# intel/QAT-ZSTD-Plugin

Measured on AMD Instinct MI355X. Metric: input MB/s via ZSTD_compress2 L1 128KiB blocks @1/2/4/8 GPU; ratio vs sw zstd, higher is better.
Workload: dtype u8

## Files before the change

include/qzstd_hip.h:

```cpp
#ifndef QZSTD_HIP_H
#define QZSTD_HIP_H

#include <stddef.h>
#include <stdint.h>

#if defined(__cplusplus)
extern "C" {
#endif

#define QZSTD_HIP_BLOCK_MAX (1u << 17)
#define QZSTD_HIP_NSEQ_ERROR 0xFFFFFFFFu
#define QZSTD_HIP_SRC_ALIGN 16u

typedef struct {
    uint32_t tableSize;
    uint32_t tileLog;
    uint32_t capLen;
    uint32_t minMatch;
    uint32_t farLog1;
    uint32_t farLog2;
    uint32_t lazy;
    uint32_t backExt;
    uint32_t nearTab;
    uint32_t window;
// ... 54 lines not shown
int qzstd_hip_stream_sync(int device, void *stream);
int qzstd_hip_stream_query(int device, void *stream);
int qzstd_hip_stream_wait(int device, void *stream, unsigned timeoutMs);
int qzstd_hip_memcpy_h2d(int device, void *stream, void *dst, const void *src, size_t bytes);
int qzstd_hip_copy_in(int device, void *stream, void *dst, const void *src_dev, size_t bytes);
int qzstd_hip_memcpy_d2h(int device, void *stream, void *dst, const void *src, size_t bytes);
int qzstd_hip_memset(int device, void *stream, void *dst, int value, size_t bytes);
int qzstd_hip_memcpy2d_d2h(int device, void *stream, void *dst, size_t dpitch, const void *src, size_t spitch,
                           size_t width, size_t height);

size_t qzstd_hip_workspace_bytes(int level, uint32_t nBlocks, uint32_t maxBlockLen);
int qzstd_hip_find_sequences(int device, void *stream, int level, const void *d_src,
                             const qzstd_hip_block_t *d_blocks, uint32_t nBlocks,
                             uint32_t maxBlockLen, void *d_seqs, uint32_t *d_nseq,
                             void *d_work, size_t workBytes);

int qzstd_hip_occupancy(int device, int level);

#define QZSTD_HIP_NSEQ_REJECTED 0xFFFFFFFEu
#define QZSTD_HIP_NSEQ_STAGING 0xFFFFFFFCu
int qzstd_hip_service_progressive(int device);
#define QZSTD_HIP_SVC_MAX_ITEMS 32u
#define QZSTD_HIP_SVC_MAX_SLOTS 1024u
typedef struct {
    const void *hSrc;
    void *dSrc;
    void *hSeqs;
    uint32_t *hCount;
    uint32_t srcLen, itemBytes, nItems, seqCapPerItem;
    uint32_t slot;
// ... 25 lines not shown
```

qat-zstd-plugin_amd/csrc/qzstd_kernels.hip:

```cpp
#include <hip/hip_runtime.h>

#include <stdint.h>
#include <stdio.h>
#include <stdlib.h>
#include <string.h>

#include <atomic>
#include <mutex>
#include <sched.h>
#include <time.h>

#include "qzstd_hip.h"
#include "qzstd_hip_internal.h"

#define QZ_PRIO(n) do { if (!CHAIN) __builtin_amdgcn_s_setprio(n); } while (0)

#ifndef QZ_PARSE_SPLIT
#define QZ_PARSE_SPLIT 3
#endif
#ifndef QZ_LINKS_PER_STEP
#define QZ_LINKS_PER_STEP 4
#endif
#ifndef QZ_WAVES_PER_EU
#define QZ_WAVES_PER_EU 5
#endif
#define QZ_OCCUPANCY __attribute__((amdgpu_waves_per_eu(QZ_WAVES_PER_EU)))

#ifdef QZ_DEBUG_DUMP
#define QZ_PLAP(acc) { const u64 tN = __builtin_amdgcn_s_memtime(); acc += tN - tQ; tQ = tN; }
#define QZ_LAP(acc) { const u64 tN = __builtin_amdgcn_s_memtime(); acc += tN - tP; tP = tN; }
#define QZ_CLAP(k) { const u64 tN = __builtin_amdgcn_s_memtime(); dC[k] += tN - tC; tC = tN; }
#else
#define QZ_PLAP(acc)
#define QZ_LAP(acc)
#define QZ_CLAP(k)
#endif

namespace {

constexpr int kMatchWaves = 8;
constexpr int kMatchThreads = kMatchWaves * 64;
// ... 689 lines not shown
}

struct HistShare {
    uint32_t *flags;
    uint32_t item;
    uint32_t epoch;
    uint32_t spinLimit;
    uint32_t nItems;
    uint32_t *tabFlags;
    uint32_t *linkFlags;
    uint32_t *tabs;
};
constexpr uint32_t kSvcTabStride = QZ_CHAIN_TABLE;
static_assert((uint32_t)kMatchWaves * kPvStride <= QZ_CHAIN_TABLE, "the deferred parse's eight windows of parse words must fit in the head table (QZ_CHAIN_TABLE)");

template <bool HAS_LONG, bool REP, bool CHAIN, bool TURNS, bool NEAR, bool DEFER = false>
__device__ __forceinline__ uint32_t qz_item(const LaunchArgs &args, const qzstd_hip_block_t &blk, const uint8_t *gsrc, uint4 *out,
                                            uint4 *chainB, uint32_t *p1B, const HistShare hsh)
{
    extern __shared__ __attribute__((aligned(16))) uint8_t smem[];
    const uint32_t tid = threadIdx.x;
    const uint32_t lane = tid & 63u;
    const uint32_t wave = rdfirst(tid >> 6);
    const bool matcher = wave < (uint32_t)kMatchWaves;
    const uint32_t n = blk.srcLen;
    const qzstd_hip_profile_t pf = args.prof;
    const uint32_t nh = n >= pf.hashBytes ? n - pf.hashBytes + 1u : 0u;
    const uint32_t nTiles = (nh + kTile - 1u) >> kTileLog;
    const uint32_t itEnd = (DEFER && !CHAIN) ? nTiles : nTiles + kLagT;
    static_assert(kNear + kLagT * kTile + 4u <= kRing - kLook, "the ring no longer holds a near source when its tile is parsed / emitted");
    const uint32_t tabShift = (uint32_t)__builtin_clz(pf.tableSize) + 1u, longShift = pf.longSize ? (uint32_t)__builtin_clz(pf.longSize) + 1u : 31u;
    const uint32_t firstTile = blk.parseFrom >> kTileLog;
    if (blk.parseFrom != 0u && (pf.segLog == 0u || (blk.parseFrom & ((1u << pf.segLog) - 1u)) != 0u || blk.parseFrom >= n)) {
        return QZSTD_HIP_NSEQ_ERROR;
    }
    if (NEAR && n > kRing) return QZSTD_HIP_NSEQ_ERROR;
    if (DEFER && args.pwWords != 0u && ((n + kTile - 1u) & ~(kTile - 1u)) > args.pwWords) return QZSTD_HIP_NSEQ_ERROR;
    if (DEFER && CHAIN && args.chainEntries != 0u && ((n + kTile - 1u) & ~(kTile - 1u)) * kEQ > args.chainEntries) return QZSTD_HIP_NSEQ_ERROR;

    uint8_t *smemI = (uint8_t *)(__attribute__((address_space(3))) uint8_t *)kLdsBase;
    if ((uint32_t)(uintptr_t)(__attribute__((address_space(3))) uint8_t *)smem != 0u) {
        return QZSTD_HIP_NSEQ_ERROR;
    }
    uint32_t *ring32 = reinterpret_cast<uint32_t *>(smemI);
    uint4 *ring128 = reinterpret_cast<uint4 *>(smemI);
    uint32_t *tbl = reinterpret_cast<uint32_t *>(smemI + kRing + kMirror);
    uint32_t *tblL = tbl + pf.tableSize;
    uint32_t *nearTab = tblL + pf.longSize;
    uint32_t *srec = nearTab + kTile;
    uint32_t *pv = srec + kLagT * kWin * kSrecWords;
    uint32_t *turnCtr = pv + kLagT * kPvStride;
    uint32_t *P1odd = turnCtr + QZSTD_HIP_LDS_CTRL / 4u;
    const uint4 *g128 = reinterpret_cast<const uint4 *>(gsrc);
    Src src;
    src.ring = (LdsWords)ring32;
    src.g = (HbmWords)reinterpret_cast<const uint32_t *>(gsrc);
    src.nearLimit = NEAR ? 0xFFFFFFFFu : kNear;
    const uint32_t nPad = (n + 15u) & ~15u;

    const uint32_t itBegin = firstTile;
    const uint32_t histEnd = itBegin << kTileLog;
    const uint32_t hi = umin(nPad, histEnd + kLook + (itBegin ? 0u : kTile));
    const uint32_t lo = hi > kRing ? (hi - kRing + 15u) & ~15u : 0u;
    constexpr uint32_t kStep = (uint32_t)kThreads * 16u;
    const uint32_t hashEnd = CHAIN ? 0u : histEnd;
    uint32_t fo = (hashEnd ? 0u : lo) + tid * 16u;
    uint4 fa0 = make_uint4(0u, 0u, 0u, 0u), fb0 = fa0, fa1 = fa0, fb1 = fa0;
    if (fo < hi) { fa0 = g128[fo >> 4]; if (fo < hashEnd) fb0 = g128[(fo >> 4) + 1u]; }
    if (fo + kStep < hi) { fa1 = g128[(fo + kStep) >> 4]; if (fo + kStep < hashEnd) fb1 = g128[((fo + kStep) >> 4) + 1u]; }
    for (uint32_t i = tid; i < pf.tableSize + pf.longSize; i += kThreads) tbl[i] = 0u;
    if (!(CHAIN && itBegin != 0u)) {
        for (uint32_t i = tid; i < kTile; i += kThreads) nearTab[i] = 0xFFFFFFFFu;
        for (uint32_t i = tid; i < kLagT * kWin * kSrecWords + kLagT * kPvStride + QZSTD_HIP_LDS_CTRL / 4u; i += kThreads) srec[i] = 0u;
    }
    const bool sharedHist = CHAIN && hsh.flags != nullptr && hsh.nItems > 1u && pf.tableSize <= kSvcTabStride;
    if (itBegin != 0u || sharedHist) __syncthreads();
    if (sharedHist) {
        constexpr uint32_t kGroup = 4096u;
        uint32_t *hist = ring32;
        uint32_t *link = ring32 + kGroup;
        const uint32_t a0 = blk.parseFrom, b0 = n, k = hsh.item;
        auto wait_for = [&](uint32_t *fl) -> bool {
            if (wave == 0u) {
                uint32_t spins = 0u, ok = 1u;
// ... 229 lines not shown
                __builtin_amdgcn_fence(__ATOMIC_ACQUIRE, "agent");
                if (lane == 0u) turnCtr[2] = ok;
            }
            __syncthreads();
            if (rdfirst(turnCtr[2]) == 0u) return QZSTD_HIP_NSEQ_ERROR;
        }
        __syncthreads();
        for (uint32_t i = tid; i < kTile; i += kThreads) nearTab[i] = 0xFFFFFFFFu;
        for (uint32_t i = tid; i < kLagT * kWin * kSrecWords + kLagT * kPvStride + QZSTD_HIP_LDS_CTRL / 4u; i += kThreads) srec[i] = 0u;
    }
    {
        const uint32_t hiMaskH = pf.hashBytes >= 8 ? 0xFFFFFFFFu : ((1u << (8u * (pf.hashBytes - 4u))) - 1u);
        for (; fo < hi; fo += kStep) {
            uint4 fa2 = make_uint4(0u, 0u, 0u, 0u), fb2 = fa2;
            const uint32_t o2 = fo + 2u * kStep;
            if (o2 < hi) { fa2 = g128[o2 >> 4]; if (o2 < hashEnd) fb2 = g128[(o2 >> 4) + 1u]; }
            if (fo >= lo) {
                const uint32_t r = ring_dw(fo) << 2;
                ring128[r >> 4] = fa0;
                if (r < kMirror) ring128[(kRing + r) >> 4] = fa0;
            }
            if (fo < hashEnd) {
                const uint32_t W[6] = { fa0.x, fa0.y, fa0.z, fa0.w, fb0.x, fb0.y };
                const uint32_t segEc = seg_end(pf, fo, n);
#pragma unroll
                for (uint32_t k = 0; k < 16u; k++) {
                    const uint32_t p = fo + k;
                    if (p + pf.hashBytes <= segEc) {
                        const uint32_t v = __builtin_amdgcn_alignbyte(W[(k >> 2) + 1u], W[k >> 2], k & 3u);
                        const uint32_t w = __builtin_amdgcn_alignbyte(W[(k >> 2) + 2u], W[(k >> 2) + 1u], k & 3u);
                        const uint32_t mixH = (v * kPrime1) ^ __umul24(pf.hashBytes > 4 ? w & hiMaskH : 0u, kPrime2 & 0xFFFFFFu);
                        atomicMax(&tbl[mixH >> tabShift], ((p + 1u) << kTagBits) | ((mixH >> 3) & kTagMask));
                        if (HAS_LONG && p + 8u <= segEc) {
                            const uint32_t m8 = (v * kPrime1) ^ (w * kPrime2);
                            atomicMax(&tblL[m8 >> longShift], ((p + 1u) << kTagBits) | ((m8 >> 3) & kTagMask));
                        }
                    }
                }
            }
            fa0 = fa1; fb0 = fb1; fa1 = fa2; fb1 = fb2;
        }
        if (itBegin != 0u && TURNS && !CHAIN && tid == 0u) *turnCtr = itBegin * (uint32_t)kMatchWaves;
        if (itBegin == 0u)
            for (uint32_t o = hi + tid * 16u; o < kTile + kLook; o += kThreads * 16u) {
                ring128[o >> 4] = make_uint4(0u, 0u, 0u, 0u);
                if (o < kMirror) ring128[(kRing + o) >> 4] = make_uint4(0u, 0u, 0u, 0u);
            }
    }
    __syncthreads();

    if (DEFER && !matcher) __builtin_amdgcn_endpgm();
    if (!matcher) {
        if (!QZ_ABLATED(32u)) __builtin_amdgcn_s_setprio(3);
        constexpr uint32_t kSplit = QZ_PARSE_SPLIT;
#ifdef QZ_DEBUG_DUMP
        u64 pI1 = 0, pW1 = 0, pI2 = 0, pW2 = 0, tQ = __builtin_amdgcn_s_memtime();
#endif
        uint32_t nseqEnd, anchorEnd;
        if (REP) {
            RepState st = { blk.parseFrom, blk.parseFrom, 0u, 0u, 0u, 0u, pf.segLog ? blk.parseFrom >> pf.segLog : 0u };
            for (uint32_t it = itBegin; it < itEnd; it++) {
                const bool work = it >= 1u && it - 1u < nTiles && it - 1u >= firstTile && !QZ_ABLATED(1u);
                const uint32_t k = it - 1u, base = k << kTileLog;
// ... 99 lines not shown
            }
            const u64 startMask = __ballot(start);
            const uint32_t smLo = (uint32_t)startMask, smHi = (uint32_t)(startMask >> 32);
            const uint32_t keepLo = lane < 32u ? smLo & (0xFFFFFFFFu << (lane & 31u)) : 0u;
            const uint32_t keepHi = lane < 32u ? smHi : smHi & (0xFFFFFFFFu << (lane & 31u));
            const uint32_t ns = umin(umin(first_diff_bit(keepLo), first_diff_bit(keepHi) | 32u), 64u);
            const bool capped = cl == pf.capLen;
            const uint32_t endj = lane + cl;
            const uint32_t nsEnd = (uint32_t)__shfl((int)ns, (int)(endj & 63u));
            uint32_t nx = endj >= 64u ? endj : nsEnd;
            nx = capped ? kNxCapped : nx;
            const uint32_t gRep = take ? 4u * cl + 32u - (31u - (uint32_t)__builtin_clz(off + 1u)) : 0u;
            if (DEFER) p1B[(tileIdx << kTileLog) + tid] = gRep | (off << 10);
            else pv[(tileIdx % kLagT) * kPvStride + tid] = REP ? (gRep | (off << 10)) : pack_pos(nx, ns, capped ? off : cl);
    };
    for (uint32_t it = itBegin; it < itEnd; it++) {
        const uint32_t t0 = it << kTileLog;
        const uint32_t p = t0 + tid;
        const uint32_t stamp = (nTilesMax - 1u - (it & (nTilesMax - 1u))) << stampShift;
        uint32_t mix = 0, old = 0;
        const uint32_t segE = rdfirst(seg_end(pf, t0, n));
        const bool valid = it < nTiles && p < nh && p + pf.hashBytes <= segE;
        const bool history = it < firstTile;

        QZ_PRIO(2);
        if (CHAIN && DEFER && wave == 0u && it == itBegin && it < nTiles)
            chain_insert_tile(pf, src, tbl, (it & 1u) ? P1odd : nearTab, it << kTileLog, n, nh, lane, args.orderedLds != 0u);
        uint32_t own[5];
        load_dw_r<5>(src, p, rp, false, own);
        uint4 fresh;
        asm volatile("" : "=v"(fresh.x), "=v"(fresh.y), "=v"(fresh.z), "=v"(fresh.w));
        const uint32_t fpos = t0 + kLook + (tid - 64u) * 16u;
        const bool refill = wave == 1u && it >= 1u && lane < kTile / 16u && fpos < nPad;
        if (refill) fresh = g128[fpos >> 4];
        if (!DEFER && it >= kLagT + firstTile && !QZ_ABLATED(8u))
            emit_window<REP>(pf, src, srec + ((it % kLagT) * kWin + wave) * kSrecWords, pv + (it % kLagT) * kPvStride + 64u * wave,
                             offH[kLagT - 1u], lenH[kLagT - 1u], t0 - kLagT * kTile + 64u * wave, ring_back(rp, kLagT * kTile), lane, out, blk.seqCap,
                             REP ? srec[(it % kLagT) * kWin * kSrecWords] : 0u, blk.mark);
        QZ_PRIO(1);
        uint32_t slot = 0, nslot = 0, slotL = 0, oldL = 0, tagL = 0;
        const bool validL = HAS_LONG && valid && p + 8u <= segE;
        uint32_t oa[4];
#pragma unroll
        for (int i = 0; i < 4; i++) oa[i] = __builtin_amdgcn_alignbyte(own[i + 1], own[i], p & 3u);
        if (valid) {
            const uint32_t v = oa[0];
            uint32_t hi = 0;
            if (pf.hashBytes > 4) hi = oa[1] & hiMask;
// ... 6 lines not shown
                const uint32_t m8 = (v * kPrime1) ^ (oa[1] * kPrime2);
                slotL = m8 >> longShift;
                tagL = (m8 >> 3) & kTagMask;
                if (!TURNS) oldL = tblL[slotL];
            }
        }
        uint32_t pre[kEL];
#pragma unroll
        for (uint32_t j = 0; j < kEL; j++) pre[j] = 0u;
        if (CHAIN && it != itBegin) {
            old = valid ? ((it & 1u) ? P1odd : nearTab)[tid] : 0u;
            if (old != 0u && (old >> kTagBits) - 1u < t0) entryOf((old >> kTagBits) - 1u, pre);
        }
        if (CHAIN && it > itBegin && it - 1u < nTiles && it - 1u >= firstTile && !QZ_ABLATED(4u)) write_flags(it - 1u, lenH[0], offH[0]);
        QZ_LAP(dI1)
        __syncthreads();
        QZ_LAP(dW1)

        QZ_PRIO(2);
        if (CHAIN && DEFER && wave == 0u && it + 1u < nTiles)
            chain_insert_tile(pf, src, tbl, ((it + 1u) & 1u) ? P1odd : nearTab, (it + 1u) << kTileLog, n, nh, lane, args.orderedLds != 0u);
        if (refill) {
            const uint32_t o = ring_dw(fpos) << 2;
            ring128[o >> 4] = fresh;
            if (o < kMirror) ring128[(kRing + o) >> 4] = fresh;
        }
        uint32_t cl = 0, off = 0;
        if (CHAIN) {
            const uint32_t *P1T = (it & 1u) ? P1odd : nearTab;
            const uint32_t tag = (mix >> 3) & kTagMask;
#ifdef QZ_DEBUG_DUMP
            tC = __builtin_amdgcn_s_memtime();
#endif
            uint32_t E[kEL];
#pragma unroll
            for (uint32_t j = 0; j < kEL; j++) E[j] = 0u;
// ... 169 lines not shown
            }
            QZ_PRIO(0);
            l1 = umin(l1, cap); l2 = umin(l2, cap); l3 = umin(l3, cap);
            if (l1 >= 4u) { cl = l1; off = p - q1; }
            if (l3 >= 4u && l3 > cl) { cl = l3; off = p - q3; }
            if (l2 >= 4u && l2 >= cl) { cl = l2; off = p - q2; }
            }
        }
        }
        if (!CHAIN && it < nTiles && !history && !QZ_ABLATED(4u)) write_flags(it, cl, off);
#pragma unroll
        for (uint32_t i = kLagT - 1u; i > 0u; i--) { offH[i] = offH[i - 1u]; lenH[i] = lenH[i - 1u]; }
        offH[0] = off;
        lenH[0] = cl;
        rp = ring_fwd(rp, kTile);
        QZ_LAP(dI2)
        if (DEFER && !CHAIN) QZ_BARRIER_LDS(); else __syncthreads();
        QZ_LAP(dW2)
    }
#ifdef QZ_DEBUG_DUMP
    if (!(blk.mark & QZSTD_HIP_MARK_COMPACT)) {
    if (lane == 0) out[blk.seqCap - 3u - wave] = make_uint4((uint32_t)dI1, (uint32_t)dW1, (uint32_t)dI2, (uint32_t)dW2);
    if (lane == 0) out[blk.seqCap - 24u - 2u * wave] = make_uint4((uint32_t)(dC[0] >> 4), (uint32_t)(dC[1] >> 4), (uint32_t)(dC[2] >> 4), (uint32_t)(dC[3] >> 4));
    if (lane == 0) out[blk.seqCap - 25u - 2u * wave] = make_uint4((uint32_t)(dC[4] >> 4), (uint32_t)dC[5], 0u, 0u);
    if (lane == 0) out[blk.seqCap - 12u - wave] = make_uint4(__builtin_amdgcn_s_getreg((4 << 0) | (0 << 6) | (31 << 11)), 0u, 0u, 0u);
    }
#endif
    if constexpr (!DEFER) return 0u;
    }

    if constexpr (DEFER && !REP) {
        constexpr uint32_t kSegLog = 12u, kSeg = 1u << kSegLog, kMaxSegs = QZSTD_HIP_BLOCK_MAX >> kSegLog;
        static_assert(kMaxSegs <= 64u, "one lane per segment in the prefix step");
// ... 195 lines not shown
                }
                total += all;
                anchorCarry = anchorOut;
            }
            __syncthreads();
        }
        if (wave != 0u) return 0u;
        uint32_t count = total + 1u;
        if (lane == 0 && total < blk.seqCap) store_entry(out, total, 0u, n - anchorCarry, 0u, blk.mark);
        if (count + 1u >= blk.seqCap) count = QZSTD_HIP_NSEQ_ERROR;
        return count;
    }
    return 0u;
}

template <bool HAS_LONG, bool REP, bool CHAIN, bool TURNS, bool NEAR>
__global__ __launch_bounds__(kThreads) QZ_OCCUPANCY void qzstd_find_sequences_kernel(LaunchArgs args)
{
    const qzstd_hip_block_t blk = args.blocks[blockIdx.x];
    const uint32_t count = qz_item<HAS_LONG, REP, CHAIN, TURNS, NEAR, true>(args, blk, args.src + blk.srcOff, args.seqs + blk.seqOff,
                                                              CHAIN ? args.chain + (size_t)blockIdx.x * args.chainStride : nullptr,
                                                              reinterpret_cast<uint32_t *>(args.chain + (size_t)blockIdx.x * args.chainStride + args.chainEntries),
                                                              HistShare{ nullptr, 0u, 0u, 0u, 0u, nullptr, nullptr, nullptr });
    asm volatile("s_waitcnt vmcnt(0)" ::: "memory");
    __syncthreads();
    if (threadIdx.x == 0u)
        __hip_atomic_store(args.nseq + blockIdx.x, count, __ATOMIC_RELEASE, __HIP_MEMORY_SCOPE_SYSTEM);
}

constexpr uint32_t kSvcQueue = 4096u;
constexpr uint32_t kSvcRing = 256u;
constexpr uint32_t kSvcMaxItems = 32u;
constexpr uint32_t kSvcSlots = 1024u;
constexpr uint32_t kSvcRejected = 0xFFFFFFFEu;

struct SvcDev {
    u64 items[kSvcQueue][8];
    uint32_t head;
// ... 324 lines not shown
            sched_yield();
        }
    }
    return 0;
}

#define QZ_SEARCHES(X, last)                                                                                    \
    X(false, false, false, false, last), X(false, true, false, false, last),        \
    X(false, false, false, true, last), X(false, true, false, true, last),                \
    X(false, false, true, true, last), X(false, true, true, true, last),      \
    X(true, false, false, false, last), X(true, true, false, false, last)
#define QZ_K(L, R, C, T, N) reinterpret_cast<const void *>(qzstd_find_sequences_kernel<L, R, C, T, N>)
#define QZ_W(L, R, C, T, M) reinterpret_cast<const void *>(qzstd_service_worker<L, R, C, T, M>)
const void *const kLaunchKernels[16] = { QZ_SEARCHES(QZ_K, false), QZ_SEARCHES(QZ_K, true) };
const void *const kWorkers[8] = { QZ_SEARCHES(QZ_W, false) };
#undef QZ_K
#undef QZ_W
#undef QZ_SEARCHES

int variant_index(const qzstd_hip_profile_t &p, bool nearK)
{
    const int search = p.chainDepth ? 2 : (p.longSize ? 3 : (p.subTileLog ? 1 : 0));
    return (nearK ? 8 : 0) + 2 * search + (p.repWin ? 1 : 0);
}

}

SvcFreeze::SvcFreeze()
{
    g_svcFreeze.fetch_add(1);
// ... 21 lines not shown
    const char *force = getenv("QZSTD_HIP_ORDERED_LDS");
    uint32_t *dBad = nullptr, hBad = 1u;
    if (!(force && atoi(force) == 0) && hipSetDevice(physDev) == hipSuccess && hipMalloc(&dBad, sizeof(uint32_t)) == hipSuccess) {
        if (hipMemset(dBad, 0, sizeof(uint32_t)) == hipSuccess) {
            hipLaunchKernelGGL(qzstd_probe_lds_order, dim3(512), dim3(kThreads), 0, 0, dBad);
            if (hipGetLastError() == hipSuccess && hipMemcpy(&hBad, dBad, sizeof(uint32_t), hipMemcpyDeviceToHost) == hipSuccess)
                verdict = hBad == 0u;
        }
        (void)hipFree(dBad);
    }
    (void)hipGetLastError();
    __atomic_store_n(&g_ldsOrdered[device], verdict + 1, __ATOMIC_RELEASE);
    return verdict;
}

extern "C" {

int qzstd_hip_find_sequences(int device, void *stream, int level, const void *d_src,
                             const qzstd_hip_block_t *d_blocks, uint32_t nBlocks, uint32_t maxBlockLen,
                             void *d_seqs, uint32_t *d_nseq, void *d_work, size_t workBytes)
{
    LaunchArgs a;
    if (nBlocks == 0) return 0;
    if (!d_src || !d_blocks || !d_seqs || !d_nseq) return fail_msg("qzstd_hip_find_sequences: null pointer");
    if (maxBlockLen > QZSTD_HIP_BLOCK_MAX) return fail_msg("qzstd_hip_find_sequences: block larger than 128 KiB");
    if (qzstd_hip_profile_for_level(level, maxBlockLen, &a.prof))
        return fail_msg("qzstd_hip_find_sequences: level outside 1..12 (optionally | QZSTD_HIP_LEVEL_REPCODES)");
    if (a.prof.tileLog != kTileLog || a.prof.extLog < 8 || a.prof.extLog > 15 || a.prof.capLen > 48 || a.prof.capLen < 32 ||
        a.prof.minMatch < 4 || a.prof.hashBytes < 4 || a.prof.hashBytes > 8 || a.prof.repWin > 16 || a.prof.chainDepth > 64 ||
        a.prof.lazy > 4 || (a.prof.subTileLog != 0u && a.prof.subTileLog != 6u) || (a.prof.segLog != 0u && (a.prof.segLog < kTileLog || a.prof.segLog > 17u)) ||
        (a.prof.chainDepth && (a.prof.subTileLog != 6u || a.prof.longSize || a.prof.nearTab)) || (a.prof.longSize && a.prof.subTileLog))
        return fail_msg("qzstd_hip_find_sequences: unsupported profile");
    const size_t lds = qzstd_hip_lds_bytes(level, maxBlockLen);
    if (lds == 0) return fail_msg("qzstd_hip_find_sequences: LDS budget exceeded");
    QZ_SET_DEVICE(device);
// ... 7 lines not shown
    }
    {
        static std::mutex attrMu;
        static bool attrDone[64];
        std::lock_guard<std::mutex> g(attrMu);
        if (phys(device) < 0) return fail_msg("qzstd_hip_find_sequences: device index out of range");
        if (!attrDone[device]) {
            size_t most = 0;
            for (int l = 1; l <= 12; l++) {
                const size_t b = qzstd_hip_lds_bytes(l, QZSTD_HIP_BLOCK_MAX);
                if (b > most) most = b;
            }
            for (const void *f : kLaunchKernels)
                QZ_CHECK(hipFuncSetAttribute(f, hipFuncAttributeMaxDynamicSharedMemorySize, (int)most),
                         "hipFuncSetAttribute(MaxDynamicSharedMemorySize)");
            attrDone[device] = true;
        }
    }
    a.chain = nullptr;
    a.pwWords = 0;
    a.chainStride = 0;
    a.chainEntries = 0;
    a.orderedLds = 0;
    if (a.prof.chainDepth) {
        a.orderedLds = (uint32_t)probe_lds_order(device, phys(device));
        const size_t need = qzstd_hip_workspace_bytes(level, nBlocks, maxBlockLen);
        if (!d_work || workBytes < need) return fail_msg("qzstd_hip_find_sequences: workspace missing or too small (qzstd_hip_workspace_bytes)");
        a.chain = static_cast<uint4 *>(d_work);
        a.chainStride = (uint32_t)(need / nBlocks / sizeof(uint4));
        a.chainEntries = (uint32_t)(need / nBlocks / (4u * QZSTD_HIP_CHAIN_ENTRY_LINKS + 4u)) * kEQ;
// ... 7 lines not shown
    if (a.prof.segLog != 12u) return fail_msg("qzstd_hip_find_sequences: unsupported profile (the deferred parse of a launch works on 4 KiB segments)");
    a.src = static_cast<const uint8_t *>(d_src);
    a.blocks = d_blocks;
    a.seqs = static_cast<uint4 *>(d_seqs);
    a.nseq = d_nseq;
#ifdef QZ_DEBUG_DUMP
    { const char *ab = getenv("QZSTD_HIP_ABLATE"); a.dbg = ab ? (uint32_t)atoi(ab) : 0u; }
#endif
#ifdef QZ_DEBUG_DUMP
    size_t ldsLaunch = lds;
    { const char *pad = getenv("QZSTD_HIP_LDS_PAD"); if (pad) ldsLaunch += (size_t)atoi(pad); }
#else
    const size_t ldsLaunch = lds;
#endif
    const dim3 grid(nBlocks), wg(kThreads);
    const void *kernel = kLaunchKernels[variant_index(a.prof, maxBlockLen <= kRing)];
    void *kargs[1] = { &a };
    if (!a.prof.chainDepth && ((a.prof.tableSize & (a.prof.tableSize - 1u)) != 0u || (a.prof.longSize & (a.prof.longSize - 1u)) != 0u || a.prof.hashBytes > 7u))
        return fail_msg("qzstd_hip_find_sequences: unsupported profile (tables below the chain levels are powers of two, hashBytes <= 7)");
    QZ_CHECK(hipLaunchKernel(kernel, grid, wg, kargs, ldsLaunch, (hipStream_t)stream), "launch qzstd_find_sequences_kernel");
    QZ_CHECK(hipGetLastError(), "launch qzstd_find_sequences_kernel");
    if (big && bigLock.owns_lock()) {
        Service &sv = g_svc[device];
        int k = sv.bigNext;
        for (int tries = 0; tries < Service::kBig && sv.bigUsed[k]; tries++) {
            if (hipEventQuery(sv.bigEv[k]) != hipErrorNotReady) { (void)hipGetLastError(); sv.bigUsed[k] = false; break; }
            k = (k + 1) % Service::kBig;
        }
        if (sv.bigUsed[k]) { (void)hipEventSynchronize(sv.bigEv[k]); (void)hipGetLastError(); }
        sv.bigNext = (k + 1) % Service::kBig;
        if (!sv.bigEv[k] && hipEventCreateWithFlags(&sv.bigEv[k], hipEventDisableTiming) != hipSuccess) { sv.bigEv[k] = nullptr; (void)hipGetLastError(); }
        if (sv.bigEv[k] && hipEventRecord(sv.bigEv[k], (hipStream_t)stream) == hipSuccess) { sv.bigUsed[k] = true; sv.bigLds[k] = lds; }
        else (void)hipGetLastError();
    }
    return 0;
}

int qzstd_hip_occupancy(int device, int level)
{
    qzstd_hip_profile_t p;
    if (qzstd_hip_profile_for_level(level, QZSTD_HIP_BLOCK_MAX, &p)) return fail_msg("qzstd_hip_occupancy: bad level");
    const size_t lds = qzstd_hip_lds_bytes(level, QZSTD_HIP_BLOCK_MAX);
    QZ_SET_DEVICE(device);
    const void *k = kLaunchKernels[variant_index(p, false)];
    (void)hipFuncSetAttribute(k, hipFuncAttributeMaxDynamicSharedMemorySize, (int)lds);
    int n = 0;
    QZ_CHECK(hipOccupancyMaxActiveBlocksPerMultiprocessor(&n, k, kThreads, lds), "hipOccupancyMaxActiveBlocksPerMultiprocessor");
    return n;
}

// ... 295 lines not shown
```

qat-zstd-plugin_amd/host/qatseqprod.c:

```c
#ifndef _GNU_SOURCE
#define _GNU_SOURCE
#endif
#include "qatseqprod.h"
#include "qzstd_hip.h"

#include <fcntl.h>
#include <pthread.h>
#include <sched.h>
#include <stdint.h>
#include <stdio.h>
#include <stdlib.h>
#include <string.h>
#include <emmintrin.h>
#include <sys/prctl.h>
#include <sys/syscall.h>
#include <sys/types.h>
#include <time.h>
#include <unistd.h>

#ifndef DEBUGLEVEL
#define DEBUGLEVEL 0
#endif

#define QZ_LEVEL_MIN 1
// ... 105 lines not shown
    int svcItemBytes;
    int svcSpinUs;
    unsigned long devBlocks[QZ_MAX_DEVICES][3];
    pthread_mutex_t mutex;
    int numa;
    int numaThreadNode;
    int devNode[QZ_MAX_DEVICES];
    unsigned int nodeNext[QZ_NUMA_NODES_MAX], anyNext;
    int svcSpinSet;
    int liveStates;
    struct QZSTD_Batcher_S *hb;
    int hintBatches;
    unsigned int gen;
    int hintCompact;
    int stageNt;
    int hintDirect;
} QZSTD_Process_T;

static QZSTD_Process_T gProc = { .status = QZSTD_FAIL, .coalesce = 1, .timeoutMs = QZ_DEFAULT_TIMEOUT_MS, .splitBlocks = 1, .service = 1,
                                 .svcItemBytes = 4096, .svcSpinUs = 400, .mutex = PTHREAD_MUTEX_INITIALIZER, .numa = 1, .numaThreadNode = -1,
                                 .hintBatches = 4 };

#define QZ_HINT_MAX_BYTES ((size_t)16 << 20)
#define QZ_HINT_PITCH ((size_t)16384)
#define QZ_HINT_PARTS 16
#define QZ_COUNT_PENDING 0xFFFFFFFDu
#define QZ_HINTS 4
#define QZ_CONTENT_LOOKUP_BLOCKS 256u
typedef struct {
    int st;
    int dev, area;
// ... 1047 lines not shown
    a->stuck = 0;
    bt->open = k;
    return k;
}

static void qzAreaRetire(QZSTD_Batcher_T *bt, int ai)
{
    QZSTD_Area_T *a = &bt->area[ai];
    int k;
    if (a->stuck) qzOrphanArea(a, bt->device, a->stream >= 0 ? bt->str[a->stream].stream : NULL);
    for (k = 0; k < QZ_HB_STREAMS_MAX; k++)
        if (bt->str[k].last == ai && !bt->str[k].stuck) bt->str[k].last = -1;
    a->st = QZ_AREA_FREE;
}

static int qzLaunchArea(QZSTD_Session_T *s, QZSTD_Batcher_T *bt, QZSTD_Area_T *a, QZSTD_BStream_T *q)
{
    const int dev = bt->device;
    const size_t work = qzstd_hip_workspace_bytes(a->level, a->nBlocks, (unsigned int)a->block);
    unsigned long t0;
    int direct, rc;
    if (!q->stream && !(q->stream = qzstd_hip_stream_create(dev))) return -1;
    if (work && !(q->dWork = qzGrowDev(dev, q->dWork, &q->dWorkCap, work))) return -1;
    direct = gProc.hintDirect == 1 || (gProc.hintDirect == 2 && work == 0);
    if (!direct) {
        if (!q->dSrc && !(q->dSrc = (unsigned char *)qzstd_hip_malloc(dev, QZ_HB_SRC_BYTES))) return -1;
        t0 = qzNowNs();
        rc = gProc.hintDirect != 3 ? qzstd_hip_copy_in(dev, q->stream, q->dSrc, a->dvSrc, a->srcUsed)
                                   : qzstd_hip_memcpy_h2d(dev, q->stream, q->dSrc, a->hSrc, a->srcUsed);
        if (s) s->hintCopyCallNs += qzNowNs() - t0;
        if (rc) return -1;
    }
    t0 = qzNowNs();
    rc = qzstd_hip_find_sequences(dev, q->stream, a->level, direct ? a->dvSrc : q->dSrc, (const qzstd_hip_block_t *)a->dvDesc, a->nBlocks,
                                  (unsigned int)a->block, a->dvSeqs, (unsigned int *)a->dvCount, q->dWork, q->dWorkCap);
    if (s) s->hintLaunchCallNs += qzNowNs() - t0;
    if (rc) return -1;
    __atomic_fetch_add(&gProc.devBlocks[dev][0], (unsigned long)a->nBlocks, __ATOMIC_RELAXED);
    __atomic_fetch_add(&bt->launches, 1ul, __ATOMIC_RELAXED);
    __atomic_fetch_add(&bt->blocks, (unsigned long)a->nBlocks, __ATOMIC_RELAXED);
    return 0;
}

static void qzAreaFailCounts(QZSTD_Area_T *a)
{
    memset(a->hCount, 0xFF, a->nBlocks * sizeof(unsigned int));
}

static void qzIssueOpen(QZSTD_Session_T *s, QZSTD_Batcher_T *bt, int force, int want)
{
// ... 604 lines not shown
    pthread_mutex_lock(&gProc.mutex);
    {
        const char *dbg = getenv("QZSTD_HIP_DEBUG");
        const char *rep = getenv("QZSTD_HIP_EXT_REPCODES");
        if (dbg && *dbg) qzLogLevel = atoi(dbg);
        gProc.levelFlags = (rep && atoi(rep) > 0) ? QZSTD_HIP_LEVEL_REPCODES : 0;
        gProc.timeoutMs = qzEnvInt("QZSTD_HIP_TIMEOUT_MS", QZ_DEFAULT_TIMEOUT_MS, 1, 600000);
        gProc.splitBlocks = qzEnvInt("QZSTD_HIP_SPLIT_BLOCKS", 1, 0, 1);
        gProc.service = qzEnvInt("QZSTD_HIP_SERVICE", 1, 0, 1);
        gProc.svcItemBytes = qzEnvInt("QZSTD_HIP_SERVICE_ITEM", 4096, 4096, (int)QZSTD_HIP_BLOCK_MAX) & ~4095;
        gProc.svcSpinUs = qzEnvInt("QZSTD_HIP_SERVICE_SPIN_US", 400, 0, 1000000);
        gProc.svcSpinSet = getenv("QZSTD_HIP_SERVICE_SPIN_US") != NULL;
        gProc.hintCompact = qzEnvInt("QZSTD_HIP_HINT_COMPACT", 1, 0, 1);
        gProc.hintBatches = qzEnvInt("QZSTD_HIP_HINT_BATCHES", 4, 1, QZ_HB_STREAMS_MAX);
        gProc.stageNt = qzEnvInt("QZSTD_HIP_STAGE_NT", 1, 0, 1);
        gProc.hintDirect = qzEnvInt("QZSTD_HIP_HINT_DIRECT", 0, 0, 3);
        (void)qzUsableCores();
    }
    if (gProc.status == QZSTD_FAIL) {
        gProc.status = qzstd_hip_device_count() > 0 ? QZSTD_STARTED : QZSTD_FAIL;
        if (gProc.status == QZSTD_FAIL) QZ_LOG(2, "no usable HIP device: %s\n", qzstd_hip_last_error());
    }
    if (gProc.status == QZSTD_STARTED) {
        gProc.status = qzBuildSlots() == QZSTD_OK ? QZSTD_OK : QZSTD_STARTED;
    }
    QZ_LOG(2, "start: status %d, %d device(s), %d slot(s)\n", gProc.status, gProc.numDevices, gProc.numSlots);
    status = gProc.status;
    pthread_mutex_unlock(&gProc.mutex);
    return status;
}

// ... 106 lines not shown
        pthread_mutex_unlock(&gProc.hb[d].mu);
    }
}
void qzstd_test_set_hint_epochs(void *state, unsigned int e)
{
    (void)state;
    qzstd_test_set_area_tags(e);
}
unsigned long qzstd_test_hint_launches(void)
{
    unsigned long n = 0;
    int d;
    for (d = 0; gProc.hb && d < gProc.numDevices; d++) n += __atomic_load_n(&gProc.hb[d].launches, __ATOMIC_RELAXED);
    return n;
}
void qzstd_test_set_service_epochs(unsigned int e)
{
    int i;
    for (i = 0; gProc.slots && i < gProc.numSlots; i++) gProc.slots[i].vEpoch = e & 0xFFFFFFu;
}
#endif


size_t qatSequenceProducer(void *sequenceProducerState, ZSTD_Sequence *outSeqs, size_t outSeqsCapacity,
                           const void *src, size_t srcSize, const void *dict, size_t dictSize,
                           int compressionLevel, size_t windowSize)
{
    QZSTD_Session_T *s = (QZSTD_Session_T *)sequenceProducerState;
    size_t rc;
    int order[QZ_HINTS], n, oi, dev, found;
// ... 40 lines not shown
```

Baseline: 24040.

## Land pinned host input inside the match kernel instead of a separate copy-in

For levels 1-4, the kernel now reads the block directly from pinned host memory and writes it into the device source buffer while it runs. Loads of later tile groups are staged a few iterations ahead and stored into the ring and the device buffer, and the separate refill path is disabled. This removes the separate copy-in before each launch and overlaps the PCIe reads with matching. In exchange, the kernel's progress now depends on host-memory latency, it adds vmcnt waits, and the old direct-read mode is removed.

New measurement: 23160. 3.7% lower.

```diff
diff --git a/include/qzstd_hip.h b/include/qzstd_hip.h
--- a/include/qzstd_hip.h
+++ b/include/qzstd_hip.h
@@ -92,6 +92,10 @@
                              const qzstd_hip_block_t *d_blocks, uint32_t nBlocks,
                              uint32_t maxBlockLen, void *d_seqs, uint32_t *d_nseq,
                              void *d_work, size_t workBytes);
+int qzstd_hip_find_sequences_land(int device, void *stream, int level, const void *d_pinned, void *d_land,
+                                  const qzstd_hip_block_t *d_blocks, uint32_t nBlocks,
+                                  uint32_t maxBlockLen, void *d_seqs, uint32_t *d_nseq,
+                                  void *d_work, size_t workBytes);
 
 int qzstd_hip_occupancy(int device, int level);
 
diff --git a/qat-zstd-plugin_amd/csrc/qzstd_kernels.hip b/qat-zstd-plugin_amd/csrc/qzstd_kernels.hip
--- a/qat-zstd-plugin_amd/csrc/qzstd_kernels.hip
+++ b/qat-zstd-plugin_amd/csrc/qzstd_kernels.hip
@@ -25,6 +25,9 @@
 #define QZ_WAVES_PER_EU 5
 #endif
 #define QZ_OCCUPANCY __attribute__((amdgpu_waves_per_eu(QZ_WAVES_PER_EU)))
+#ifndef QZ_LAND_D
+#define QZ_LAND_D 2
+#endif
 
 #ifdef QZ_DEBUG_DUMP
 #define QZ_PLAP(acc) { const u64 tN = __builtin_amdgcn_s_memtime(); acc += tN - tQ; tQ = tN; }
@@ -744,10 +747,11 @@
 constexpr uint32_t kSvcTabStride = QZ_CHAIN_TABLE;
 static_assert((uint32_t)kMatchWaves * kPvStride <= QZ_CHAIN_TABLE, "the deferred parse's eight windows of parse words must fit in the head table (QZ_CHAIN_TABLE)");
 
-template <bool HAS_LONG, bool REP, bool CHAIN, bool TURNS, bool NEAR, bool DEFER = false>
+template <bool HAS_LONG, bool REP, bool CHAIN, bool TURNS, bool NEAR, bool DEFER = false, bool LAND = false>
 __device__ __forceinline__ uint32_t qz_item(const LaunchArgs &args, const qzstd_hip_block_t &blk, const uint8_t *gsrc, uint4 *out,
-                                            uint4 *chainB, uint32_t *p1B, const HistShare hsh)
-{
+                                            uint4 *chainB, uint32_t *p1B, const HistShare hsh, const uint8_t *pin = nullptr)
+{
+    static_assert(!LAND || (DEFER && !CHAIN), "only the launch kernels below the chain levels land their input");
     extern __shared__ __attribute__((aligned(16))) uint8_t smem[];
     const uint32_t tid = threadIdx.x;
     const uint32_t lane = tid & 63u;
@@ -764,6 +768,7 @@
     if (blk.parseFrom != 0u && (pf.segLog == 0u || (blk.parseFrom & ((1u << pf.segLog) - 1u)) != 0u || blk.parseFrom >= n)) {
         return QZSTD_HIP_NSEQ_ERROR;
     }
+    if (LAND && blk.parseFrom != 0u) return QZSTD_HIP_NSEQ_ERROR;
     if (NEAR && n > kRing) return QZSTD_HIP_NSEQ_ERROR;
     if (DEFER && args.pwWords != 0u && ((n + kTile - 1u) & ~(kTile - 1u)) > args.pwWords) return QZSTD_HIP_NSEQ_ERROR;
     if (DEFER && CHAIN && args.chainEntries != 0u && ((n + kTile - 1u) & ~(kTile - 1u)) * kEQ > args.chainEntries) return QZSTD_HIP_NSEQ_ERROR;
@@ -782,6 +787,8 @@
     uint32_t *turnCtr = pv + kLagT * kPvStride;
     uint32_t *P1odd = turnCtr + QZSTD_HIP_LDS_CTRL / 4u;
     const uint4 *g128 = reinterpret_cast<const uint4 *>(gsrc);
+    const uint4 *in128 = LAND ? reinterpret_cast<const uint4 *>(pin) : g128;
+    uint4 *land128 = const_cast<uint4 *>(g128);
     Src src;
     src.ring = (LdsWords)ring32;
     src.g = (HbmWords)reinterpret_cast<const uint32_t *>(gsrc);
@@ -796,8 +803,8 @@
     const uint32_t hashEnd = CHAIN ? 0u : histEnd;
     uint32_t fo = (hashEnd ? 0u : lo) + tid * 16u;
     uint4 fa0 = make_uint4(0u, 0u, 0u, 0u), fb0 = fa0, fa1 = fa0, fb1 = fa0;
-    if (fo < hi) { fa0 = g128[fo >> 4]; if (fo < hashEnd) fb0 = g128[(fo >> 4) + 1u]; }
-    if (fo + kStep < hi) { fa1 = g128[(fo + kStep) >> 4]; if (fo + kStep < hashEnd) fb1 = g128[((fo + kStep) >> 4) + 1u]; }
+    if (fo < hi) { fa0 = in128[fo >> 4]; if (fo < hashEnd) fb0 = g128[(fo >> 4) + 1u]; }
+    if (fo + kStep < hi) { fa1 = in128[(fo + kStep) >> 4]; if (fo + kStep < hashEnd) fb1 = g128[((fo + kStep) >> 4) + 1u]; }
     for (uint32_t i = tid; i < pf.tableSize + pf.longSize; i += kThreads) tbl[i] = 0u;
     if (!(CHAIN && itBegin != 0u)) {
         for (uint32_t i = tid; i < kTile; i += kThreads) nearTab[i] = 0xFFFFFFFFu;
@@ -1057,11 +1064,12 @@
         for (; fo < hi; fo += kStep) {
             uint4 fa2 = make_uint4(0u, 0u, 0u, 0u), fb2 = fa2;
             const uint32_t o2 = fo + 2u * kStep;
-            if (o2 < hi) { fa2 = g128[o2 >> 4]; if (o2 < hashEnd) fb2 = g128[(o2 >> 4) + 1u]; }
+            if (o2 < hi) { fa2 = in128[o2 >> 4]; if (o2 < hashEnd) fb2 = g128[(o2 >> 4) + 1u]; }
             if (fo >= lo) {
                 const uint32_t r = ring_dw(fo) << 2;
                 ring128[r >> 4] = fa0;
                 if (r < kMirror) ring128[(kRing + r) >> 4] = fa0;
+                if constexpr (LAND) land128[fo >> 4] = fa0;
             }
             if (fo < hashEnd) {
                 const uint32_t W[6] = { fa0.x, fa0.y, fa0.z, fa0.w, fb0.x, fb0.y };
@@ -1090,6 +1098,7 @@
                 if (o < kMirror) ring128[(kRing + o) >> 4] = make_uint4(0u, 0u, 0u, 0u);
             }
     }
+    if constexpr (LAND) asm volatile("s_waitcnt vmcnt(0)" ::: "memory");
     __syncthreads();
 
     if (DEFER && !matcher) __builtin_amdgcn_endpgm();
@@ -1219,6 +1228,12 @@
             if (DEFER) p1B[(tileIdx << kTileLog) + tid] = gRep | (off << 10);
             else pv[(tileIdx % kLagT) * kPvStride + tid] = REP ? (gRep | (off << 10)) : pack_pos(nx, ns, capped ? off : cl);
     };
+    constexpr uint32_t kLandD = QZ_LAND_D, kLandGroup = (uint32_t)kMatchWaves * kTile;
+    static_assert(kLandD >= 1u && kLandD <= 6u, "a group is loaded inside the eight iterations that end with its store");
+    static_assert(kMatchWaves == 8 && 9u * kTile + 60u <= kTile + kLook, "a group is in the ring before the first tile that reads it");
+    static_assert(kNear + 2u * kTile + kLook + 4u <= kRing, "a group's store overwrites a near source of the iteration it is stored in");
+    const uint32_t nLandG = LAND ? nTiles >> 3 : 0u;
+    uint4 landed = make_uint4(0u, 0u, 0u, 0u);
     for (uint32_t it = itBegin; it < itEnd; it++) {
         const uint32_t t0 = it << kTileLog;
         const uint32_t p = t0 + tid;
@@ -1236,7 +1251,7 @@
         uint4 fresh;
         asm volatile("" : "=v"(fresh.x), "=v"(fresh.y), "=v"(fresh.z), "=v"(fresh.w));
         const uint32_t fpos = t0 + kLook + (tid - 64u) * 16u;
-        const bool refill = wave == 1u && it >= 1u && lane < kTile / 16u && fpos < nPad;
+        const bool refill = !LAND && wave == 1u && it >= 1u && lane < kTile / 16u && fpos < nPad;
         if (refill) fresh = g128[fpos >> 4];
         if (!DEFER && it >= kLagT + firstTile && !QZ_ABLATED(8u))
             emit_window<REP>(pf, src, srec + ((it % kLagT) * kWin + wave) * kSrecWords, pv + (it % kLagT) * kPvStride + 64u * wave,
@@ -1273,12 +1288,23 @@
         }
         if (CHAIN && it > itBegin && it - 1u < nTiles && it - 1u >= firstTile && !QZ_ABLATED(4u)) write_flags(it - 1u, lenH[0], offH[0]);
         QZ_LAP(dI1)
-        __syncthreads();
+        if constexpr (LAND) QZ_BARRIER_LDS(); else __syncthreads();
         QZ_LAP(dW1)
 
         QZ_PRIO(2);
         if (CHAIN && DEFER && wave == 0u && it + 1u < nTiles)
             chain_insert_tile(pf, src, tbl, ((it + 1u) & 1u) ? P1odd : nearTab, (it + 1u) << kTileLog, n, nh, lane, args.orderedLds != 0u);
+        if constexpr (LAND) {
+            if ((it & 7u) == 7u && (it >> 3) < nLandG) {
+                const uint32_t lpos = kLook + kTile + (it >> 3) * kLandGroup + wave * kTile + lane * 16u;
+                if (lane < kTile / 16u && lpos < nPad) {
+                    const uint32_t o = ring_dw(lpos) << 2;
+                    ring128[o >> 4] = landed;
+                    if (o < kMirror) ring128[(kRing + o) >> 4] = landed;
+                    land128[lpos >> 4] = landed;
+                }
+            }
+        }
         if (refill) {
             const uint32_t o = ring_dw(fpos) << 2;
             ring128[o >> 4] = fresh;
@@ -1478,9 +1504,22 @@
         offH[0] = off;
         lenH[0] = cl;
         rp = ring_fwd(rp, kTile);
+        if constexpr (LAND) {
+            const uint32_t ld = it + kLandD;
+            if ((ld & 7u) == 7u && (ld >> 3) < nLandG) {
+                asm volatile("s_waitcnt vmcnt(0)" ::: "memory");
+                const uint32_t lpos = kLook + kTile + (ld >> 3) * kLandGroup + wave * kTile + lane * 16u;
+                if (lane < kTile / 16u && lpos < nPad) landed = in128[lpos >> 4];
+            }
+        }
         QZ_LAP(dI2)
         if (DEFER && !CHAIN) QZ_BARRIER_LDS(); else __syncthreads();
         QZ_LAP(dW2)
+    }
+    if constexpr (LAND) {
+        for (uint32_t o = kLook + kTile + nLandG * kLandGroup + tid * 16u; o < nPad; o += (uint32_t)kMatchThreads * 16u) land128[o >> 4] = in128[o >> 4];
+        asm volatile("s_waitcnt vmcnt(0)" ::: "memory");
+        __syncthreads();
     }
 #ifdef QZ_DEBUG_DUMP
     if (!(blk.mark & QZSTD_HIP_MARK_COMPACT)) {
@@ -1706,14 +1745,15 @@
     return 0u;
 }
 
-template <bool HAS_LONG, bool REP, bool CHAIN, bool TURNS, bool NEAR>
-__global__ __launch_bounds__(kThreads) QZ_OCCUPANCY void qzstd_find_sequences_kernel(LaunchArgs args)
+template <bool HAS_LONG, bool REP, bool CHAIN, bool TURNS, bool NEAR, bool LAND = false>
+__global__ __launch_bounds__(kThreads) QZ_OCCUPANCY void qzstd_find_sequences_kernel(LaunchArgs args, const uint8_t *pinned)
 {
     const qzstd_hip_block_t blk = args.blocks[blockIdx.x];
-    const uint32_t count = qz_item<HAS_LONG, REP, CHAIN, TURNS, NEAR, true>(args, blk, args.src + blk.srcOff, args.seqs + blk.seqOff,
+    const uint32_t count = qz_item<HAS_LONG, REP, CHAIN, TURNS, NEAR, true, LAND>(args, blk, args.src + blk.srcOff, args.seqs + blk.seqOff,
                                                               CHAIN ? args.chain + (size_t)blockIdx.x * args.chainStride : nullptr,
                                                               reinterpret_cast<uint32_t *>(args.chain + (size_t)blockIdx.x * args.chainStride + args.chainEntries),
-                                                              HistShare{ nullptr, 0u, 0u, 0u, 0u, nullptr, nullptr, nullptr });
+                                                              HistShare{ nullptr, 0u, 0u, 0u, 0u, nullptr, nullptr, nullptr },
+                                                              LAND ? pinned + blk.srcOff : nullptr);
     asm volatile("s_waitcnt vmcnt(0)" ::: "memory");
     __syncthreads();
     if (threadIdx.x == 0u)
@@ -2068,6 +2108,9 @@
 #define QZ_W(L, R, C, T, M) reinterpret_cast<const void *>(qzstd_service_worker<L, R, C, T, M>)
 const void *const kLaunchKernels[16] = { QZ_SEARCHES(QZ_K, false), QZ_SEARCHES(QZ_K, true) };
 const void *const kWorkers[8] = { QZ_SEARCHES(QZ_W, false) };
+#define QZ_KL(L, R, C, T, N) (C ? nullptr : reinterpret_cast<const void *>(qzstd_find_sequences_kernel<L, R, false, T, N, !C>))
+const void *const kLandKernels[16] = { QZ_SEARCHES(QZ_KL, false), QZ_SEARCHES(QZ_KL, true) };
+#undef QZ_KL
 #undef QZ_K
 #undef QZ_W
 #undef QZ_SEARCHES
@@ -2119,11 +2162,9 @@
     return verdict;
 }
 
-extern "C" {
-
-int qzstd_hip_find_sequences(int device, void *stream, int level, const void *d_src,
-                             const qzstd_hip_block_t *d_blocks, uint32_t nBlocks, uint32_t maxBlockLen,
-                             void *d_seqs, uint32_t *d_nseq, void *d_work, size_t workBytes)
+static int launch_find(int device, void *stream, int level, const void *d_src, const void *pinned,
+                       const qzstd_hip_block_t *d_blocks, uint32_t nBlocks, uint32_t maxBlockLen,
+                       void *d_seqs, uint32_t *d_nseq, void *d_work, size_t workBytes)
 {
     LaunchArgs a;
     if (nBlocks == 0) return 0;
@@ -2161,6 +2202,9 @@
             for (const void *f : kLaunchKernels)
                 QZ_CHECK(hipFuncSetAttribute(f, hipFuncAttributeMaxDynamicSharedMemorySize, (int)most),
                          "hipFuncSetAttribute(MaxDynamicSharedMemorySize)");
+            for (const void *f : kLandKernels)
+                if (f) QZ_CHECK(hipFuncSetAttribute(f, hipFuncAttributeMaxDynamicSharedMemorySize, (int)most),
+                                "hipFuncSetAttribute(MaxDynamicSharedMemorySize)");
             attrDone[device] = true;
         }
     }
@@ -2198,8 +2242,9 @@
     const size_t ldsLaunch = lds;
 #endif
     const dim3 grid(nBlocks), wg(kThreads);
-    const void *kernel = kLaunchKernels[variant_index(a.prof, maxBlockLen <= kRing)];
-    void *kargs[1] = { &a };
+    const void *kernel = (pinned ? kLandKernels : kLaunchKernels)[variant_index(a.prof, maxBlockLen <= kRing)];
+    if (!kernel) return fail_msg("qzstd_hip_find_sequences_land: levels 1..4 only (the chain levels take qzstd_hip_copy_in + qzstd_hip_find_sequences)");
+    void *kargs[2] = { &a, &pinned };
     if (!a.prof.chainDepth && ((a.prof.tableSize & (a.prof.tableSize - 1u)) != 0u || (a.prof.longSize & (a.prof.longSize - 1u)) != 0u || a.prof.hashBytes > 7u))
         return fail_msg("qzstd_hip_find_sequences: unsupported profile (tables below the chain levels are powers of two, hashBytes <= 7)");
     QZ_CHECK(hipLaunchKernel(kernel, grid, wg, kargs, ldsLaunch, (hipStream_t)stream), "launch qzstd_find_sequences_kernel");
@@ -2218,6 +2263,23 @@
         else (void)hipGetLastError();
     }
     return 0;
+}
+
+extern "C" {
+
+int qzstd_hip_find_sequences(int device, void *stream, int level, const void *d_src,
+                             const qzstd_hip_block_t *d_blocks, uint32_t nBlocks, uint32_t maxBlockLen,
+                             void *d_seqs, uint32_t *d_nseq, void *d_work, size_t workBytes)
+{
+    return launch_find(device, stream, level, d_src, nullptr, d_blocks, nBlocks, maxBlockLen, d_seqs, d_nseq, d_work, workBytes);
+}
+
+int qzstd_hip_find_sequences_land(int device, void *stream, int level, const void *d_pinned, void *d_land,
+                                  const qzstd_hip_block_t *d_blocks, uint32_t nBlocks, uint32_t maxBlockLen,
+                                  void *d_seqs, uint32_t *d_nseq, void *d_work, size_t workBytes)
+{
+    if (nBlocks != 0 && !d_pinned) return fail_msg("qzstd_hip_find_sequences_land: null pointer");
+    return launch_find(device, stream, level, d_land, d_pinned, d_blocks, nBlocks, maxBlockLen, d_seqs, d_nseq, d_work, workBytes);
 }
 
 int qzstd_hip_occupancy(int device, int level)
diff --git a/qat-zstd-plugin_amd/host/qatseqprod.c b/qat-zstd-plugin_amd/host/qatseqprod.c
--- a/qat-zstd-plugin_amd/host/qatseqprod.c
+++ b/qat-zstd-plugin_amd/host/qatseqprod.c
@@ -143,7 +143,7 @@
     unsigned int gen;
     int hintCompact;
     int stageNt;
-    int hintDirect;
+    unsigned long hintCopyIns;
 } QZSTD_Process_T;
 
 static QZSTD_Process_T gProc = { .status = QZSTD_FAIL, .coalesce = 1, .timeoutMs = QZ_DEFAULT_TIMEOUT_MS, .splitBlocks = 1, .service = 1,
@@ -1221,26 +1221,32 @@
     a->st = QZ_AREA_FREE;
 }
 
+extern int qzstd_hip_find_sequences_land(int device, void *stream, int level, const void *d_pinned, void *d_land,
+                                         const qzstd_hip_block_t *d_blocks, uint32_t nBlocks, uint32_t maxBlockLen,
+                                         void *d_seqs, uint32_t *d_nseq, void *d_work, size_t workBytes) __attribute__((weak));
+
 static int qzLaunchArea(QZSTD_Session_T *s, QZSTD_Batcher_T *bt, QZSTD_Area_T *a, QZSTD_BStream_T *q)
 {
     const int dev = bt->device;
     const size_t work = qzstd_hip_workspace_bytes(a->level, a->nBlocks, (unsigned int)a->block);
+    const int land = qzstd_hip_find_sequences_land != NULL && (a->level & ~QZSTD_HIP_LEVEL_REPCODES) <= 4;
     unsigned long t0;
-    int direct, rc;
+    int rc;
     if (!q->stream && !(q->stream = qzstd_hip_stream_create(dev))) return -1;
     if (work && !(q->dWork = qzGrowDev(dev, q->dWork, &q->dWorkCap, work))) return -1;
-    direct = gProc.hintDirect == 1 || (gProc.hintDirect == 2 && work == 0);
-    if (!direct) {
-        if (!q->dSrc && !(q->dSrc = (unsigned char *)qzstd_hip_malloc(dev, QZ_HB_SRC_BYTES))) return -1;
+    if (!q->dSrc && !(q->dSrc = (unsigned char *)qzstd_hip_malloc(dev, QZ_HB_SRC_BYTES))) return -1;
+    if (!land) {
         t0 = qzNowNs();
-        rc = gProc.hintDirect != 3 ? qzstd_hip_copy_in(dev, q->stream, q->dSrc, a->dvSrc, a->srcUsed)
-                                   : qzstd_hip_memcpy_h2d(dev, q->stream, q->dSrc, a->hSrc, a->srcUsed);
+        rc = qzstd_hip_copy_in(dev, q->stream, q->dSrc, a->dvSrc, a->srcUsed);
         if (s) s->hintCopyCallNs += qzNowNs() - t0;
         if (rc) return -1;
+        __atomic_fetch_add(&gProc.hintCopyIns, 1ul, __ATOMIC_RELAXED);
     }
     t0 = qzNowNs();
-    rc = qzstd_hip_find_sequences(dev, q->stream, a->level, direct ? a->dvSrc : q->dSrc, (const qzstd_hip_block_t *)a->dvDesc, a->nBlocks,
-                                  (unsigned int)a->block, a->dvSeqs, (unsigned int *)a->dvCount, q->dWork, q->dWorkCap);
+    rc = land ? qzstd_hip_find_sequences_land(dev, q->stream, a->level, a->dvSrc, q->dSrc, (const qzstd_hip_block_t *)a->dvDesc, a->nBlocks,
+                                              (unsigned int)a->block, a->dvSeqs, (unsigned int *)a->dvCount, q->dWork, q->dWorkCap)
+              : qzstd_hip_find_sequences(dev, q->stream, a->level, q->dSrc, (const qzstd_hip_block_t *)a->dvDesc, a->nBlocks,
+                                         (unsigned int)a->block, a->dvSeqs, (unsigned int *)a->dvCount, q->dWork, q->dWorkCap);
     if (s) s->hintLaunchCallNs += qzNowNs() - t0;
     if (rc) return -1;
     __atomic_fetch_add(&gProc.devBlocks[dev][0], (unsigned long)a->nBlocks, __ATOMIC_RELAXED);
@@ -1875,7 +1881,6 @@
         gProc.hintCompact = qzEnvInt("QZSTD_HIP_HINT_COMPACT", 1, 0, 1);
         gProc.hintBatches = qzEnvInt("QZSTD_HIP_HINT_BATCHES", 4, 1, QZ_HB_STREAMS_MAX);
         gProc.stageNt = qzEnvInt("QZSTD_HIP_STAGE_NT", 1, 0, 1);
-        gProc.hintDirect = qzEnvInt("QZSTD_HIP_HINT_DIRECT", 0, 0, 3);
         (void)qzUsableCores();
     }
     if (gProc.status == QZSTD_FAIL) {
@@ -2012,6 +2017,10 @@
     for (d = 0; gProc.hb && d < gProc.numDevices; d++) n += __atomic_load_n(&gProc.hb[d].launches, __ATOMIC_RELAXED);
     return n;
 }
+unsigned long qzstd_test_hint_copy_ins(void)
+{
+    return __atomic_load_n(&gProc.hintCopyIns, __ATOMIC_RELAXED);
+}
 void qzstd_test_set_service_epochs(unsigned int e)
 {
     int i;
```
